# jnsquire/sregex

Measured on AMD Instinct MI355X. Metric: GB/s input scanned (whole job), gen-data stream resident in HBM, higher is better.
Workload: dtype u8; 1 GPU; configs[1]: /[a-z]+@[a-z]+\.[a-z]+/ Pike first-match + captures; 1 stream x 4.00 GiB gen-data (abccc.. + 'aaabbccb'); bytes_per_gpu=4294967293, streams_per_gpu=1, segment_bytes=16896, fixup_rounds=0, matches=0, engine=scan, lineage_passes=0, world_size=1

## Files before the change

### sregex_amd/csrc/sre_hip_scan.hip

```cpp
#include <hip/hip_runtime.h>
#include <stdlib.h>
#include "sre_hip_scan.h"
#include "sre_hip_streams.h"
#include "sre_hip_tile.h"

#define SRE_HIP_PIKE_COUNT 2
#define EV_DONE 1
#define EV_POP  2
#define RC_DECLINED (-5)
#define RC_ERROR    (-1)


__global__ void
sre_k_gen_data(uint8_t *__restrict__ dst, uint64_t n, uint64_t body, const uint8_t *__restrict__ tail)
{
    const uint64_t stride = (uint64_t) gridDim.x * blockDim.x * 16;
    for (uint64_t base = ((uint64_t) blockIdx.x * blockDim.x + threadIdx.x) * 16; base < n;
         base += stride)
    {
        uint8_t  v[16];
        unsigned ph = (unsigned) (base % 5);
#pragma unroll
        for (int k = 0; k < 16; k++) {
            uint64_t i = base + k;
// ... 439 lines not shown

template <int MODE, int BITS, bool WIDE, bool GROW>
__global__ __launch_bounds__(SRE_SCAN_BLOCK, MODE == SRE_HIP_PIKE_COUNT ? SRE_COUNT_BLOCKS : SRE_FIRST_BLOCKS) void
sre_k_scan(const sre_scan_tables_t *__restrict__ tabp, sre_scan_geom_t G,
           sre_seg_summary_t *__restrict__ sum, const sre_stream_status_t *__restrict__ st_lo,
           const uint8_t *__restrict__ entry)
{
    constexpr int      TILE = SRE_SCAN_ROUND;
    constexpr int      WARM = SRE_SCAN_LINE;
    constexpr int      STRIDE = 8 / BITS;
    constexpr uint32_t ROWRAW = TILE / STRIDE * (WIDE ? 2 : 1);
    constexpr uint32_t ROWB = 2 * ROWRAW + 16;
    constexpr int      GIDX = 16 / STRIDE;
    typedef const __attribute__((address_space(3))) uint32_t *lds_u32_t;
    extern __shared__ __attribute__((aligned(16))) uint8_t lds[];
    __shared__ uint16_t clsx[BITS == 8 ? 1 : 8 / BITS][256];
    __shared__ sre_scan_tables_t Ts;

    const uint32_t tid = threadIdx.x;
    const uint32_t nst = tabp->nstates, nrows = tabp->fast_rows, nsh = tabp->nshadow;
    uint32_t *fast = reinterpret_cast<uint32_t *>(lds);
    uint8_t  *clsl = lds + nrows * SRE_FAST_ROW_BYTES;
    uint8_t  *trl = clsl + 256;
    const uint32_t tr_bytes = (nst * (tabp->ncls + 1) * 2u + 15u) & ~15u;
    uint8_t  *sfl = trl + tr_bytes;
    uint8_t  *tile = lds + (((size_t) (sfl - lds) + nst + 15u) & ~(size_t) 15u);
    RowDesc  *rows = reinterpret_cast<RowDesc *>(tile + SRE_SCAN_BLOCK * ROWB);
    (void) nrows;
    if (tid == 0) {
        Ts = *tabp;
        Ts.cls = clsl;
        Ts.state_flags = sfl;
    }
    constexpr uint32_t LDS_SLOW = 1u << 16;
    constexpr uint32_t LDS_CNT_SHIFT = 24;
    constexpr uint32_t LDS_FRESH = 1u << 17;
    const uint32_t fast_lds = (uint32_t) (uintptr_t) (__attribute__((address_space(3))) uint8_t *) lds;
    const uint32_t trap_lds = fast_lds + nst * SRE_FAST_ROW_BYTES;
    const uint32_t shadow_lds = trap_lds + SRE_FAST_ROW_BYTES;
    auto to_lds = [fast_lds, trap_lds](uint32_t g) -> uint32_t {
        if (g & SRE_FAST_SLOW) return trap_lds | LDS_SLOW;
        return (fast_lds + (g & ~(SRE_FAST_ROW_BYTES - 1)))
               | (((g >> SRE_FAST_CNT_SHIFT) & SRE_FAST_CNT_MASK) << LDS_CNT_SHIFT)
               | ((MODE == SRE_HIP_PIKE_COUNT && (g & SRE_FAST_EVT)) ? (128u << LDS_CNT_SHIFT) : 0u)
               | ((MODE == SRE_HIP_PIKE_COUNT && (g & SRE_FAST_NEXT_FRESH)) ? LDS_FRESH : 0u);
    };
    for (uint32_t i = tid; i < nst * 64; i += SRE_SCAN_BLOCK) {
        uint4 e = reinterpret_cast<const uint4 *>(tabp->fast)[i];
        e.x = to_lds(e.x);
        e.y = to_lds(e.y);
        e.z = to_lds(e.z);
        e.w = to_lds(e.w);
        reinterpret_cast<uint4 *>(fast)[i] = e;
    }
    fast[nst * 256 + tid] = trap_lds | LDS_SLOW;
    for (uint32_t q = 0; q < nsh; q++) {
        const uint32_t s = tabp->shadow_state[q], addr = shadow_lds + q * SRE_FAST_ROW_BYTES;
        const uint32_t gl = tabp->fast[s * 256 + tid];
        fast[(nst + 1 + q) * 256 + tid] = (gl & SRE_FAST_STABLE) ? addr : to_lds(gl);
    }
    for (uint32_t i = tid; i < nst * (tabp->ncls + 1); i += SRE_SCAN_BLOCK) {
        reinterpret_cast<uint16_t *>(trl)[i] = tabp->trans2[i];
    }
    for (uint32_t i = tid; i < tabp->nstates; i += SRE_SCAN_BLOCK) sfl[i] = tabp->state_flags[i];
    clsl[tid] = tabp->cls[tid];
    if (BITS != 8) {
#pragma unroll
        for (int u = 0; u < 8 / BITS; u++) clsx[u][tid] = (uint16_t) ((uint32_t) tabp->cls[tid] << (BITS * u + (WIDE ? 2 : 0)));
    }
    __syncthreads();
    const sre_scan_tables_t &T = Ts;

    const uint64_t g = (uint64_t) blockIdx.x * SRE_SCAN_BLOCK + tid;
    bool           active = g < G.nsegs;
    uint32_t       sidx = 0;
    uint64_t       k = 0;
    int64_t        lo_s = -2;
    if (active) {
        uint32_t a = 0, b = G.nstreams;
        while (b - a > 1) {
            uint32_t m = (a + b) >> 1;
            if (geom_first(G, m) <= g) a = m; else b = m;
        }
        sidx = a;
        k = g - geom_first(G, a);
        if (st_lo != nullptr) {
            lo_s = st_lo[sidx].done ? -1 : st_lo[sidx].first_bad;
            if (lo_s < 0 || (int64_t) k < lo_s) active = false;
        }
    }

    Walk w;
    w.T = &T;
    w.tr2 = reinterpret_cast<const uint16_t *>(trl);
    w.data = nullptr;
    w.n = 0;
    w.st = 0;
    w.ev_kind = 0;
    w.ev_state = w.ev_sym = 0;
    w.ev_pos = w.ev_sp = -1;
    w.ev_apos = -1;
    w.ev_astate = 0;
    w.cur_sp = -1;
    w.warm_lo = 0;
    w.anchor_pos = -1;
    w.anchor_state = 0;
    w.lm_state = w.lm_sym = 0;
    w.lm_pos = w.lm_sp = w.lm_apos = -1;
    w.lm_astate = 0;
    w.count = 0;
    w.term_pos = -1;
    w.fl = 0;

    int64_t  seg_a = 0, seg_b = 0;
    uint32_t s_in = 0, seed = 0;
    int64_t  in_pe_pos = -1;
    uint32_t in_pe_state = 0, in_pe_sym = 0;
    bool     last_seg = false, warm = false;
    RowDesc mine;
    mine.addr = 0;
    mine.lo = 0;
    mine.hi16 = -1;
    if (active) {
        w.data = geom_ptr(G, sidx);
        w.n = (int64_t) geom_len(G, sidx);
        seg_a = (int64_t) k * G.seg_bytes;
        seg_b = seg_a + G.seg_bytes;
        const uint64_t nseg = geom_first(G, sidx + 1) - geom_first(G, sidx);
        last_seg = (k + 1 == nseg);
        if (seg_b > w.n) seg_b = w.n;
        if (last_seg && G.sentry != nullptr && (G.sentry[sidx] & SRE_SENTRY_NO_EOF)) w.fl |= F_NO_EOF;

        if (k == 0) {
            w.st = G.sentry != nullptr ? SRE_SENTRY_STATE(G.sentry[sidx])
                   : (G.flags & SRE_GEOM_CONTINUES) ? G.entry_state : T.init[G.init_variant];
            w.cur_sp = 0;
        } else if (lo_s >= 0 && (int64_t) k == lo_s) {
            const sre_seg_summary_t &c = sum[g - 1];
            w.st = c.s_out & ~SRE_STATE_SKIP;
            w.set(F_SKIP_NEXT, MODE == SRE_HIP_PIKE_COUNT && (c.s_out & SRE_STATE_SKIP) != 0);
            w.cur_sp = c.cur_sp;
            if (c.flags & SRE_SUM_PENDING) {
                w.fl |= F_HAS_EV;
                w.ev_state = c.pe_state;
                w.ev_sym = c.pe_sym;
                w.ev_pos = c.pe_pos;
                w.ev_sp = c.pe_sp;
                w.ev_apos = c.pe_apos;
                w.ev_astate = c.pe_astate;
                w.ev_kind = (uint8_t) (w.tr2[c.pe_state * (T.ncls + 1) + c.pe_sym] >> 8);
                if (MODE == SRE_HIP_PIKE_COUNT) {
                    w.fl |= F_IN_PENDING;
                    in_pe_pos = c.pe_pos;
                    in_pe_state = c.pe_state;
                    in_pe_sym = c.pe_sym;
                }
            }
        } else if (entry != nullptr && entry[g] != 0xffu) {
            w.st = entry[g];
            if (MODE == SRE_HIP_PIKE_COUNT && lo_s > 0 && (T.state_flags[w.st] & 1)) {
                const sre_seg_summary_t &c = sum[geom_first(G, sidx) + lo_s - 1];
                if (c.flags & SRE_SUM_PENDING) {
                    w.fl |= F_HAS_EV | F_IN_PENDING;
                    w.ev_state = c.pe_state;
                    w.ev_sym = c.pe_sym;
                    w.ev_pos = c.pe_pos;
                    w.ev_sp = c.pe_sp;
                    w.ev_apos = -1;
                    w.ev_astate = 0;
                    w.ev_kind = (uint8_t) (w.tr2[c.pe_state * (T.ncls + 1) + c.pe_sym] >> 8);
                    in_pe_pos = c.pe_pos;
                    in_pe_state = c.pe_state;
                    in_pe_sym = c.pe_sym;
                }
            }
        } else {
            warm = true;
            seed = T.init[0];
            if (lo_s > 0) {
                const sre_seg_summary_t &c = sum[geom_first(G, sidx) + lo_s - 1];
                const uint32_t           cs = c.s_out & ~SRE_STATE_SKIP;
                if (cs != 0) {
                    if (!(MODE == SRE_HIP_PIKE_COUNT && (T.state_flags[cs] & 1))) {
                        seed = cs;
                    } else if (c.flags & SRE_SUM_PENDING) {
                        seed = cs;
                        w.fl |= F_HAS_EV;
                        w.ev_state = c.pe_state;
                        w.ev_sym = c.pe_sym;
                        w.ev_pos = c.pe_pos;
                        w.ev_sp = c.pe_sp;
                        w.ev_apos = -1;
                        w.ev_astate = 0;
                        w.ev_kind = (uint8_t) (w.tr2[c.pe_state * (T.ncls + 1) + c.pe_sym] >> 8);
                    }
                }
            }
            w.st = seed;
        }
        w.warm_lo = seg_a >= (int64_t) WARM ? seg_a - (int64_t) WARM : 0;
        s_in = w.st | (MODE == SRE_HIP_PIKE_COUNT && w.f(F_SKIP_NEXT) ? SRE_STATE_SKIP : 0u);
        mine.addr = (uint64_t) reinterpret_cast<uintptr_t>(w.data) + (uint64_t) (seg_a - WARM);
        mine.lo = warm ? (seg_a >= WARM ? 0 : (int32_t) (WARM - seg_a)) : WARM;
        mine.hi16 = (int32_t) (WARM + (seg_b - seg_a)) - 16;
    }
    rows[tid] = mine;

    int64_t  fcA_pos = -1, fcB_pos = -1, fc_sp0 = -1;
    uint32_t fcA_len = 0, fcA_s0 = 0, fcB_len = 0, fcB_s0 = 0;
    int64_t  lz_pos = -1;
    uint32_t lz_s0 = 0;
    auto note_span = [&](int64_t pos, uint32_t len, uint32_t s0, uint32_t cnt, bool warm_round) {
        w.fl &= ~F_HAS_EV;
        if (warm_round) return;
        if (w.f(F_SP_DIRTY)) {
            fcA_pos = fcB_pos;
            fcA_len = fcB_len;
            fcA_s0 = fcB_s0;
        } else {
            fc_sp0 = w.cur_sp;
            fcA_pos = -1;
        }
        fcB_pos = pos;
        fcB_len = len;
        fcB_s0 = s0;
        if (w.f(F_PEND_LAZY)) {
            fcB_pos = lz_pos;
            fcB_len = len + (w.f(F_LZ_GROUP) ? 16u : (uint32_t) TILE);
            fcB_s0 = lz_s0;
        }
        w.fl |= F_SP_DIRTY;
        w.count += cnt;
    };
    constexpr bool any_fresh = GROW;
    auto fast_span_done = [&](int64_t pos, uint32_t len, uint32_t s0, uint32_t sum, bool fresh1, bool warm_round) {
        if (!any_fresh) {
            if (sum) note_span(pos, len, s0, sum, warm_round);
            return;
        }
        if (sum == 0) {
            w.fl &= ~F_PEND_LAZY;
            return;
        }
        if (sum & 127u) note_span(pos, len, s0, sum & 127u, warm_round);
        else if (sum) w.fl &= ~F_HAS_EV;
        if (fresh1) {
            w.fl |= F_PEND_LAZY;
            w.set(F_LZ_GROUP, len == 16u);
            lz_pos = pos;
            lz_s0 = s0;
        } else {
            w.fl &= ~F_PEND_LAZY;
        }
    };
    auto settle = [&]() {
        if (MODE != SRE_HIP_PIKE_COUNT || !(w.fl & (F_SP_DIRTY | F_PEND_LAZY))) return;
        if (w.f(F_SP_DIRTY)) {
            int64_t sp0 = fc_sp0;
            if (fcA_pos >= 0) sp0 = resolve_fast_span(&T, w.tr2, w.data, fcA_pos, fcA_len, fcA_s0, -1, -1, 0, 0).sp;
            const SpanResult r = resolve_fast_span(&T, w.tr2, w.data, fcB_pos, fcB_len, fcB_s0, sp0, w.ev_pos, w.ev_state, w.ev_sym);
            if (r.last_pos >= 0) {
                w.fl |= F_LM_VALID;
                w.lm_pos = r.last_pos;
                w.lm_state = r.last_state;
                w.lm_sym = r.last_sym;
                w.lm_sp = r.last_sp;
                const bool anchored = r.last_sp < fcB_pos && r.last_pos - fcB_pos <= 256 && fcB_pos >= seg_a;
                w.lm_apos = anchored ? fcB_pos : (int64_t) -1;
                w.lm_astate = anchored ? fcB_s0 : 0u;
            }
            w.cur_sp = r.sp;
            w.fl &= ~F_SP_DIRTY;
        }
        if (w.f(F_PEND_LAZY)) {
            const SpanResult r = resolve_fast_span(&T, w.tr2, w.data, lz_pos, w.f(F_LZ_GROUP) ? 16u : (uint32_t) TILE, lz_s0,
                                                   -1, -1, 0, 0);
            w.fl &= ~F_PEND_LAZY;
            if (r.pend_pos >= 0) {
                w.fl |= F_HAS_EV;
                w.ev_pos = r.pend_pos;
                w.ev_state = r.pend_state;
                w.ev_sym = r.pend_sym;
                w.ev_kind = (uint8_t) (w.tr2[r.pend_state * (T.ncls + 1) + r.pend_sym] >> 8);
                w.ev_sp = w.cur_sp;
                const bool anchored = w.cur_sp < lz_pos && lz_pos >= seg_a;
                w.ev_apos = anchored ? lz_pos : (int64_t) -1;
                w.ev_astate = anchored ? lz_s0 : 0u;
            }
        }
    };

    constexpr uint32_t SU_UNSET = 0xffffffffu;
    uint32_t           su = SU_UNSET, run_off = 0;
    static_assert(SRE_SCAN_MAX_SHADOWS == 2, "two shadow rows");
    const uint32_t sh_st0 = nsh > 0 ? tabp->shadow_state[0] : 0xffffu, sh_st1 = nsh > 1 ? tabp->shadow_state[1] : 0xffffu;
    const uint32_t sh_ad0 = shadow_lds, sh_ad1 = shadow_lds + SRE_FAST_ROW_BYTES;
    const uint32_t     two = 2;
    (void) two;

    const uint32_t nrounds = WARM / TILE + G.seg_bytes / TILE;
    const uint32_t lag = (tid >> 5) & 1u;
    constexpr uint32_t DIST = SRE_SCAN_PREFETCH;
    __syncthreads();
    auto round = [&](const uint32_t s, uint4 (&regs)[4]) __attribute__((always_inline)) {
        __builtin_amdgcn_fence(__ATOMIC_ACQ_REL, "wavefront");
        __builtin_amdgcn_wave_barrier();
        tile_store<BITS, WIDE>(regs, tile, clsx, tid, s);
        __builtin_amdgcn_fence(__ATOMIC_ACQ_REL, "wavefront");
        __builtin_amdgcn_wave_barrier();
        if (s + DIST <= nrounds) tile_fetch(regs, rows, tid, s + DIST);

        if (s < lag || s - lag >= nrounds) return;
        const uint32_t r = s - lag;
        const bool     warm_round = (r < WARM / TILE);
        if (!active || w.f(F_FINISHED) || (warm_round && !warm)) return;
        const int64_t base = seg_a - WARM + (int64_t) r * TILE;
        if (base >= seg_b || base < 0) return;
        w.anchor_pos = warm_round ? -1 : base;
        w.anchor_state = w.st;

        constexpr int ROWW = (ROWRAW + 3) / 4;
        uint32_t      roww[ROWW < 4 ? 4 : ROWW];
        {
            const uint8_t *src = tile + tid * ROWB + (r & 1u) * ROWRAW;
            if (ROWW >= 4) {
#pragma unroll
                for (int x = 0; x < ROWW / 4; x++) {
                    const uint4 v = *reinterpret_cast<const uint4 *>(src + 16 * x);
                    roww[4 * x] = v.x; roww[4 * x + 1] = v.y; roww[4 * x + 2] = v.z; roww[4 * x + 3] = v.w;
                }
            } else if (ROWW == 2) {
                const uint2 v = *reinterpret_cast<const uint2 *>(src);
                roww[0] = v.x; roww[1] = v.y;
            } else {
                roww[0] = *reinterpret_cast<const uint32_t *>(src);
            }
        }
        if (base + TILE <= seg_b && !(MODE == SRE_HIP_PIKE_COUNT && w.f(F_SKIP_NEXT))) {
            uint32_t t = fast_lds + w.st * SRE_FAST_ROW_BYTES, cnt = 0;
            if (MODE != SRE_HIP_PIKE_COUNT && !warm_round) {
                const uint32_t sha = w.st == sh_st0 ? sh_ad0 : w.st == sh_st1 ? sh_ad1 : 0u;
                if (!w.f(F_SHADOW)) {
                    if (sha) {
                        w.fl |= F_SHADOW;
                        run_off = (uint32_t) (base - seg_a);
                    } else if (su == SU_UNSET) {
                        su = (uint32_t) (base - seg_a);
                    }
                }
                if (w.f(F_SHADOW)) t = sha;
            }
#pragma unroll
            for (int j = 0; j < TILE * BITS / 8; j++) {
                uint32_t a;
                if (WIDE) {
                    a = (j & 1) ? add_w0_w<1>(t, roww[j >> 1]) : add_w0_w<0>(t, roww[j >> 1]);
                } else {
                    const uint32_t wj = roww[j >> 2];
                    const uint32_t ix = (j & 3) == 0 ? byte_x4<0>(wj, two) : (j & 3) == 1 ? byte_x4<1>(wj, two)
                                      : (j & 3) == 2 ? byte_x4<2>(wj, two) : byte_x4<3>(wj, two);
                    a = add_w0_w<2>(t, ix);
                }
                t = *(lds_u32_t) (uintptr_t) a;
                if (MODE == SRE_HIP_PIKE_COUNT) cnt = add_b3(cnt, t);
            }
            if (!(t & LDS_SLOW)) {
                const uint32_t ridx = ((t & 0xffffu) - fast_lds) / SRE_FAST_ROW_BYTES;
                if (MODE == SRE_HIP_PIKE_COUNT) fast_span_done(base, TILE, w.st, cnt, (t & LDS_FRESH) != 0, warm_round);
                w.st = MODE == SRE_HIP_PIKE_COUNT ? ridx : ridx <= nst ? ridx : ridx == nst + 1 ? sh_st0 : sh_st1;
                if (MODE != SRE_HIP_PIKE_COUNT && w.f(F_SHADOW) && ridx <= nst) {
                    w.fl &= ~F_SHADOW;
                    if (su == SU_UNSET) su = (uint32_t) (base - seg_a);
                }
                if (r + 1 == WARM / TILE) {
                    s_in = w.st | (MODE == SRE_HIP_PIKE_COUNT && w.f(F_SKIP_NEXT) ? SRE_STATE_SKIP : 0u);
                    settle();
                    w.cur_sp = -1;
                    if (w.f(F_HAS_EV)) w.ev_sp = -1;
                    if (w.st == 0) w.fl |= F_FINISHED;
                    if (MODE == SRE_HIP_PIKE_COUNT) {
                        w.set(F_IN_PENDING, w.f(F_HAS_EV));
                        in_pe_pos = w.ev_pos;
                        in_pe_state = w.ev_state;
                        in_pe_sym = w.ev_sym;
                    }
                }
                return;
            }
        }
        if (MODE != SRE_HIP_PIKE_COUNT && !warm_round) {
            w.fl &= ~F_SHADOW;
            if (su == SU_UNSET) su = (uint32_t) (base - seg_a);
        }
#pragma unroll 1
        for (uint32_t q = 0; q < TILE / 16; q++) {
            const int64_t gp = base + q * 16;
            if (gp >= seg_b || w.f(F_FINISHED)) break;
            const int64_t g_end = gp + 16 <= seg_b ? gp + 16 : seg_b;
            bool          exact = (g_end != gp + 16) || (MODE == SRE_HIP_PIKE_COUNT && w.f(F_SKIP_NEXT));
            uint32_t      t = fast_lds + w.st * SRE_FAST_ROW_BYTES, cnt = 0;
            if (!exact) {
                constexpr int GW = GIDX * (WIDE ? 2 : 1) / 4;
                uint32_t      gw[GW];
                const uint32_t *gsrc = reinterpret_cast<const uint32_t *>(tile + tid * ROWB + (r & 1u) * ROWRAW) + q * GW;
#pragma unroll
                for (int x = 0; x < GW; x++) gw[x] = gsrc[x];
#pragma unroll
                for (int j = 0; j < GIDX; j++) {
                    const uint32_t ix = WIDE ? (gw[j >> 1] >> ((j & 1) * 16)) & 0xffffu
                                             : ((gw[j >> 2] >> ((j & 3) * 8)) & 0xffu) << 2;
                    t = *(lds_u32_t) (uintptr_t) ((t & 0xffffu) + ix);
                    if (MODE == SRE_HIP_PIKE_COUNT) cnt += t >> LDS_CNT_SHIFT;
                }
                exact = (t & LDS_SLOW) != 0;
            }
            if (exact) {
                settle();
                slow_run<MODE>(w, gp, g_end, warm_round, seed);
            } else {
                const uint32_t st1 = ((t & 0xffffu) - fast_lds) / SRE_FAST_ROW_BYTES;
                if (MODE == SRE_HIP_PIKE_COUNT) fast_span_done(gp, 16, w.st, cnt, (t & LDS_FRESH) != 0, warm_round);
                w.st = st1;
            }
        }
        if (r + 1 == WARM / TILE) {
            s_in = w.st | (MODE == SRE_HIP_PIKE_COUNT && w.f(F_SKIP_NEXT) ? SRE_STATE_SKIP : 0u);
            settle();
            w.cur_sp = -1;
            if (w.f(F_HAS_EV)) w.ev_sp = -1;
            if (w.st == 0) w.fl |= F_FINISHED;
            if (MODE == SRE_HIP_PIKE_COUNT) {
                w.set(F_IN_PENDING, w.f(F_HAS_EV));
                in_pe_pos = w.ev_pos;
                in_pe_state = w.ev_state;
                in_pe_sym = w.ev_sym;
            }
        }
    
    };
    uint4 regs[4];
    tile_fetch(regs, rows, tid, 0);
    if (DIST == 1) {
        for (uint32_t s = 0; s <= nrounds; s++) round(s, regs);
    } else {
        uint4 regs2[4];
        if (nrounds >= 1) tile_fetch(regs2, rows, tid, 1);
        for (uint32_t s = 0; s <= nrounds; s += 2) {
            round(s, regs);
            if (s + 1 <= nrounds) round(s + 1, regs2);
        }
    }

    if (!active) return;

    if (last_seg && !w.f(F_FINISHED) && !(G.flags & SRE_GEOM_NO_EOF) && !w.f(F_NO_EOF)) {
        settle();
        w.anchor_pos = -1;
        slow_run<MODE>(w, w.n, w.n + 1, false, 0);
    }
    settle();

    sre_seg_summary_t out;
    {
        const uint32_t seg_len = (uint32_t) (seg_b - seg_a);
        if (MODE == SRE_HIP_PIKE_COUNT || (w.f(F_FINISHED) && su == SU_UNSET)) su = 0;
        out.stable_until = su == SU_UNSET ? seg_len : su;
        out.stable_from = (MODE != SRE_HIP_PIKE_COUNT && w.f(F_SHADOW)) ? run_off : seg_len;
    }
    out.s_in = w.f(F_UNRESOLVED) ? 0xffffffffu : s_in;
    out.s_out = w.st | (MODE == SRE_HIP_PIKE_COUNT && w.f(F_SKIP_NEXT) ? SRE_STATE_SKIP : 0u);
    out.flags = 0;
    out.pad = 0;
    out.count = w.count;
    out.term_pos = w.term_pos;
    out.cur_sp = w.cur_sp;
    if (w.f(F_FINISHED) && w.term_pos >= 0) out.flags |= SRE_SUM_TERM;
    if (w.f(F_ERROR)) out.flags |= SRE_SUM_ERROR;
    if (w.f(F_HAS_EV)) out.flags |= SRE_SUM_PENDING;
    if (w.f(F_LM_VALID)) out.flags |= SRE_SUM_LASTEV;
    if (MODE == SRE_HIP_PIKE_COUNT && w.f(F_IN_PENDING)) out.flags |= SRE_SUM_IN_PENDING;
    if (MODE != SRE_HIP_PIKE_COUNT && out.stable_until == G.seg_bytes && !last_seg) out.flags |= SRE_SUM_STABLE;
    out.in_pe_pos = in_pe_pos;
    out.in_pe_state = in_pe_state;
    out.in_pe_sym = in_pe_sym;
    out.pe_state = w.ev_state;
    out.pe_sym = w.ev_sym;
    out.pe_pos = w.ev_pos;
    out.pe_sp = w.ev_sp;
    out.lm_state = w.lm_state;
    out.lm_sym = w.lm_sym;
    out.lm_pos = w.lm_pos;
    out.lm_sp = w.lm_sp;
    out.lm_apos = w.lm_apos;
    out.lm_astate = w.lm_astate;
    out.pe_apos = w.ev_apos;
    out.pe_astate = w.ev_astate;
    sum[g] = out;
    if (MODE != SRE_HIP_PIKE_COUNT && G.digest != nullptr) {
        sre_seg_digest_t dg;
        dg.s_in = out.s_in;
        dg.s_out = out.s_out;
        dg.bits = ((out.flags & SRE_SUM_TERM) ? 2u : 0u) | ((out.flags & SRE_SUM_LASTEV) ? 4u : 0u) | (out.cur_sp >= 0 ? 8u : 0u)
                  | ((out.flags & SRE_SUM_STABLE) ? 0u : 16u);
        dg.count = (uint32_t) out.count;
        G.digest[g] = dg;
    }
}


#define SRE_FN_CHUNK 256u

template <int BITS>
__global__ __launch_bounds__(256) void
sre_k_seg_functions(const sre_scan_tables_t *__restrict__ tabp, sre_scan_geom_t G,
                    const sre_stream_status_t *__restrict__ status, uint8_t *__restrict__ fn)
{
    constexpr int STRIDE = 8 / BITS;
    constexpr int GIDX = 16 / STRIDE;
    typedef const __attribute__((address_space(3))) uint32_t *lds_u32_t;
    extern __shared__ __attribute__((aligned(16))) uint8_t lds[];
    __shared__ uint16_t clsx[BITS == 8 ? 1 : 8 / BITS][256];
    const uint32_t tid = threadIdx.x, nst = tabp->nstates, nsym = tabp->ncls + 1;
    uint32_t *fast = reinterpret_cast<uint32_t *>(lds);
    uint8_t  *clsl = lds + (nst + 1) * SRE_FAST_ROW_BYTES;
    uint16_t *tr2 = reinterpret_cast<uint16_t *>(clsl + 256);
    constexpr uint32_t LDS_SLOW = 1u << 16;
    const uint32_t fast_lds = (uint32_t) (uintptr_t) (__attribute__((address_space(3))) uint8_t *) lds;
    const uint32_t trap_lds = fast_lds + nst * SRE_FAST_ROW_BYTES;
    for (uint32_t i = tid; i < nst * 256; i += 256) {
        const uint32_t gl = tabp->fast[i];
        fast[i] = (gl & SRE_FAST_SLOW) ? (trap_lds | LDS_SLOW) : fast_lds + (gl & ~(SRE_FAST_ROW_BYTES - 1));
    }
    fast[nst * 256 + tid] = trap_lds | LDS_SLOW;
    clsl[tid] = tabp->cls[tid];
    for (uint32_t i = tid; i < nst * nsym; i += 256) tr2[i] = tabp->trans2[i];
    if (BITS != 8) {
#pragma unroll
        for (int u = 0; u < 8 / BITS; u++) clsx[u][tid] = (uint16_t) ((uint32_t) tabp->cls[tid] << (BITS * u + 2));
    }
    __syncthreads();

    const uint32_t lane = tid & 63u;
    const uint64_t g = (uint64_t) blockIdx.x * 4 + (tid >> 6);
    if (g >= G.nsegs) return;
    const uint32_t s = stream_of(G, g);
    const uint64_t k = g - geom_first(G, s);
    if (status[s].done || (int64_t) k < status[s].first_bad) return;
    if (lane >= nst) {
        fn[g * 64 + lane] = 0;
        return;
    }
    const uint8_t *data = geom_ptr(G, s);
    const int64_t  n = (int64_t) geom_len(G, s);
    int64_t        p = (int64_t) k * G.seg_bytes, seg_b = p + G.seg_bytes;
    if (seg_b > n) seg_b = n;
    uint32_t cur = lane;
    const bool count_mode = tabp->mode == SRE_HIP_PIKE_COUNT;
    auto exact = [&](int64_t from, int64_t to) {
        if (!count_mode) {
            for (int64_t q = from; q < to; q++) cur = tr2[cur * nsym + clsl[data[q]]] & 0xffu;
            return;
        }
        int64_t  pend = -1;
        uint32_t pkind = 0, guard = 0;
        for (int64_t q = from; q < to; q++) {
            const uint32_t sym = clsl[data[q]];
            const uint32_t t2 = tr2[cur * nsym + sym];
            if (t2 >> 8) {
                pend = q;
                pkind = t2 >> 8;
            }
            cur = t2 & 0xffu;
            if (cur != 0) continue;
            int64_t sp = q + 1;
            if (pend >= 0) {
                const bool    pop = pkind == EV_POP || pkind == SRE_DEV_EV_POP_FULL;
                const bool    empty = pkind == EV_POP || pkind == SRE_DEV_EV_DONE_EMPTY;
                const int64_t e = pop ? pend : pend + 1;
                sp = empty ? e + 1 : e;
            } else if (++guard < 2) {
                sp = q;
            }
            if (pend >= 0) guard = 0;
            if (sp < 1) sp = 1;
            if (sp > n) sp = n;
            cur = tabp->init[restart_variant_of(*tabp, data[sp - 1])];
            pend = -1;
            q = sp - 1;
        }
    };
    for (; p + 16 <= seg_b; p += 16) {
        const sre_u32x4 v = *reinterpret_cast<const __attribute__((address_space(1))) sre_u32x4_unaligned *>(
            reinterpret_cast<uintptr_t>(data + p));
        const uint32_t words[4] = {v.x, v.y, v.z, v.w};
        uint32_t       t = fast_lds + cur * SRE_FAST_ROW_BYTES;
#pragma unroll
        for (int j = 0; j < GIDX; j++) {
            uint32_t ix = 0;
#pragma unroll
            for (int u = 0; u < STRIDE; u++) {
                const int      b = j * STRIDE + u;
                const uint32_t c = (words[b >> 2] >> ((b & 3) * 8)) & 0xffu;
                ix |= BITS == 8 ? c << 2 : (uint32_t) clsx[u][c];
            }
            t = *(lds_u32_t) (uintptr_t) ((t & 0xffffu) + ix);
        }
        if (t & LDS_SLOW) exact(p, p + 16);
        else cur = ((t & 0xffffu) - fast_lds) / SRE_FAST_ROW_BYTES;
    }
    exact(p, seg_b);
    fn[g * 64 + lane] = (uint8_t) cur;
}

// ... 1769 lines not shown
```

### sregex_amd/csrc/sre_hip_tile.h

```cpp
#ifndef SRE_HIP_TILE_H
#define SRE_HIP_TILE_H

#include <hip/hip_runtime.h>
#include "sre_hip_scan.h"

namespace {

struct __attribute__((aligned(16))) RowDesc {
    uint64_t addr;
    int32_t  lo;
    int32_t  hi16;
};

typedef uint32_t sre_u32x4 __attribute__((ext_vector_type(4)));
typedef sre_u32x4 __attribute__((aligned(1))) sre_u32x4_unaligned;

__device__ inline void
tile_fetch(uint4 (&regs)[4], const RowDesc *rows, uint32_t tid, uint32_t stage)
{
    const uint32_t wbase = (tid & ~63u) + (stage & 1u) * 32u, lane = tid & 63u;
    const int32_t  line_off = (int32_t) ((stage >> 1) * SRE_SCAN_LINE);
#pragma unroll
    for (uint32_t i = 0; i < 4; i++) {
        const uint32_t piece = i * 64 + lane;
        const uint32_t row = wbase + piece / 8, col = piece % 8;
        const int32_t  off = line_off + (int32_t) (col * 16);
        const uint4    d = *reinterpret_cast<const uint4 *>(&rows[row]);
        sre_u32x4      v = {0, 0, 0, 0};
        if ((off >= (int32_t) d.z) & (off <= (int32_t) d.w)) {
            const uint64_t a = (((uint64_t) d.y << 32) | d.x) + (uint64_t) (int64_t) off;
            v = *reinterpret_cast<const __attribute__((address_space(1))) sre_u32x4_unaligned *>(a);
        }
        regs[i] = make_uint4(v.x, v.y, v.z, v.w);
    }
}

template <int BITS, bool WIDE>
__device__ inline void
tile_store(const uint4 (&regs)[4], uint8_t *tile, const uint16_t (*clsx)[256], uint32_t tid, uint32_t stage)
{
    constexpr int      STRIDE = 8 / BITS;
    constexpr uint32_t HALFB = SRE_SCAN_ROUND / STRIDE * (WIDE ? 2 : 1);
    constexpr uint32_t ROWB = 2 * HALFB + 16;
    constexpr uint32_t PIECEB = HALFB / 4;
    const uint32_t wbase = (tid & ~63u) + (stage & 1u) * 32u, lane = tid & 63u;
#pragma unroll
    for (uint32_t i = 0; i < 4; i++) {
        const uint32_t piece = i * 64 + lane;
        const uint32_t row = wbase + piece / 8, col = piece % 8;
        const uint32_t words[4] = {regs[i].x, regs[i].y, regs[i].z, regs[i].w};
        uint8_t       *dst = tile + row * ROWB + col * PIECEB;
        if (BITS == 8) {
            *reinterpret_cast<uint4 *>(dst) = regs[i];
        } else {
            constexpr int NIDX = 16 / STRIDE;
            constexpr int PERW = WIDE ? 2 : 4;
            uint32_t      out[NIDX / PERW];
#pragma unroll
            for (int k = 0; k < NIDX; k++) {
                uint32_t v = 0;
#pragma unroll
                for (int u = 0; u < STRIDE; u++) {
                    const int      b = k * STRIDE + u;
                    const uint32_t c = (words[b >> 2] >> ((b & 3) * 8)) & 0xffu;
                    v |= (uint32_t) clsx[u][c];
                }
                if (k % PERW) out[k / PERW] |= v << ((k % PERW) * (32 / PERW)); else out[k / PERW] = v;
            }
            constexpr int NW = NIDX / PERW;
            if (PIECEB == 4) *reinterpret_cast<uint32_t *>(dst) = out[0];
            else if (PIECEB == 8) *reinterpret_cast<uint2 *>(dst) = make_uint2(out[0], out[1 % NW]);
            else *reinterpret_cast<uint4 *>(dst) = make_uint4(out[0], out[1 % NW], out[2 % NW], out[3 % NW]);
        }
    }
}

constexpr uint32_t SRE_TILE2_ROWB = SRE_SCAN_ROUND + 16;

__device__ inline void
tile2_fetch(uint4 (&regs)[4], const RowDesc *rows, uint32_t tid, uint32_t stage)
{
    const uint32_t wbase = (tid & ~63u) + (stage & 1u) * 32u, lane = tid & 63u;
    const int32_t  line_off = (int32_t) ((stage >> 1) * SRE_SCAN_LINE);
#pragma unroll
    for (uint32_t i = 0; i < 4; i++) {
        const uint32_t row = wbase + (lane >> 2) + 16u * (i >> 1), col = (lane & 3u) + 4u * (i & 1u);
        const int32_t  off = line_off + (int32_t) (col * 16);
        const uint4    d = *reinterpret_cast<const uint4 *>(&rows[row]);
        sre_u32x4      v = {0, 0, 0, 0};
        if ((off >= (int32_t) d.z) & (off <= (int32_t) d.w)) {
            const uint64_t a = (((uint64_t) d.y << 32) | d.x) + (uint64_t) (int64_t) off;
            v = *reinterpret_cast<const __attribute__((address_space(1))) sre_u32x4_unaligned *>(a);
        }
        regs[i] = make_uint4(v.x, v.y, v.z, v.w);
    }
}

__device__ inline void
tile2_store(const uint4 (&regs)[4], uint4 (&hold)[2], uint8_t *tile, uint32_t tid, uint32_t stage)
{
    const uint32_t wave = tid & ~63u, lane = tid & 63u, h = stage & 1u;
    const uint32_t rnew = wave + h * 32u + (lane >> 2), rold = wave + (1u - h) * 32u + (lane >> 2);
    const uint32_t col = (lane & 3u) * 16u;
    *reinterpret_cast<uint4 *>(tile + rnew * SRE_TILE2_ROWB + col) = regs[0];
    *reinterpret_cast<uint4 *>(tile + (rnew + 16u) * SRE_TILE2_ROWB + col) = regs[2];
    *reinterpret_cast<uint4 *>(tile + rold * SRE_TILE2_ROWB + col) = hold[0];
    *reinterpret_cast<uint4 *>(tile + (rold + 16u) * SRE_TILE2_ROWB + col) = hold[1];
    hold[0] = regs[1];
    hold[1] = regs[3];
}

}

#endif
```

Before: 5458 GB/s.

## Add uniform-stride fast path for tile fetch and OR3 class packing in tile store

Adds a per-wave setup that detects when the 64 rows a wave reads are evenly strided from a common base. For the stages where every piece is in bounds, a simplified fetch replaces the per-piece row-descriptor loads and bounds checks with scalar base plus stride addressing. It also adds a specialised tile_store path for 2-bit wide tables that combines class lookups with v_or3_b32. This cuts per-round VALU and LDS-descriptor work, but adds setup cost, register pressure and a second fetch code path.

Result: slower. 5312 GB/s (-2.7%).

```diff
diff --git a/sregex_amd/csrc/sre_hip_scan.hip b/sregex_amd/csrc/sre_hip_scan.hip
--- a/sregex_amd/csrc/sre_hip_scan.hip
+++ b/sregex_amd/csrc/sre_hip_scan.hip
@@ -765,13 +765,19 @@
     const uint32_t lag = (tid >> 5) & 1u;
     constexpr uint32_t DIST = SRE_SCAN_PREFETCH;
     __syncthreads();
+    constexpr bool MID = MODE != SRE_HIP_PIKE_COUNT && BITS == 2 && WIDE;
+    TileMid        mid;
+    if (MID) tile_mid_setup(mid, rows, tid);
     auto round = [&](const uint32_t s, uint4 (&regs)[4]) __attribute__((always_inline)) {
         __builtin_amdgcn_fence(__ATOMIC_ACQ_REL, "wavefront");
         __builtin_amdgcn_wave_barrier();
-        tile_store<BITS, WIDE>(regs, tile, clsx, tid, s);
+        tile_store<BITS, WIDE, MID>(regs, tile, clsx, tid, s);
         __builtin_amdgcn_fence(__ATOMIC_ACQ_REL, "wavefront");
         __builtin_amdgcn_wave_barrier();
-        if (s + DIST <= nrounds) tile_fetch(regs, rows, tid, s + DIST);
+        if (s + DIST <= nrounds) {
+            if (MID && tile_mid_stage(mid, s + DIST)) tile_fetch_mid(regs, mid, s + DIST);
+            else tile_fetch(regs, rows, tid, s + DIST);
+        }
 
         if (s < lag || s - lag >= nrounds) return;
         const uint32_t r = s - lag;
diff --git a/sregex_amd/csrc/sre_hip_tile.h b/sregex_amd/csrc/sre_hip_tile.h
--- a/sregex_amd/csrc/sre_hip_tile.h
+++ b/sregex_amd/csrc/sre_hip_tile.h
@@ -35,7 +35,93 @@
     }
 }
 
-template <int BITS, bool WIDE>
+struct TileMid {
+    uint64_t base;
+    uint32_t d8;
+    uint32_t s_first, s_count;
+    uint32_t off;
+};
+
+__device__ inline uint64_t
+tile_uniform64(uint64_t v)
+{
+    const uint32_t lo = (uint32_t) __builtin_amdgcn_readfirstlane((int) (uint32_t) v);
+    const uint32_t hi = (uint32_t) __builtin_amdgcn_readfirstlane((int) (uint32_t) (v >> 32));
+    return ((uint64_t) hi << 32) | lo;
+}
+
+__device__ inline void
+tile_mid_setup(TileMid &m, const RowDesc *rows, uint32_t tid)
+{
+    const uint32_t wave = tid & ~63u, lane = tid & 63u;
+    const int32_t  c16 = (int32_t) ((lane & 7u) * 16u);
+    int32_t        lf = 0, ll = 0x7fffffff;
+    uint64_t       a[8];
+#pragma unroll
+    for (uint32_t q = 0; q < 8; q++) {
+        const uint4   d = *reinterpret_cast<const uint4 *>(&rows[wave + q * 8u + (lane >> 3)]);
+        const int32_t lo = (int32_t) d.z, hi = (int32_t) d.w;
+        const int32_t f = lo > c16 ? (lo - c16 + (int32_t) SRE_SCAN_LINE - 1) / (int32_t) SRE_SCAN_LINE : 0;
+        const int32_t l = hi >= c16 ? (hi - c16) / (int32_t) SRE_SCAN_LINE : -1;
+        lf = f > lf ? f : lf;
+        ll = l < ll ? l : ll;
+        a[q] = (((uint64_t) d.y << 32) | d.x) + (uint64_t) (int64_t) c16;
+    }
+    uint64_t base = a[0];
+#pragma unroll
+    for (int x = 32; x >= 1; x >>= 1) {
+        const uint64_t o = ((uint64_t) (uint32_t) __shfl_xor((int) (base >> 32), x) << 32) | (uint32_t) __shfl_xor((int) base, x);
+        const int32_t  of = __shfl_xor(lf, x), ol = __shfl_xor(ll, x);
+        base = o < base ? o : base;
+        lf = of > lf ? of : lf;
+        ll = ol < ll ? ol : ll;
+    }
+    const uint64_t d0 = a[1] - a[0];
+    const uint64_t d8 = tile_uniform64(d0);
+    bool ok = (d8 >> 28) == 0 && ((a[0] - base) >> 31) == 0;
+#pragma unroll
+    for (uint32_t q = 1; q < 8; q++) ok = ok && a[q] == a[0] + q * d8;
+    if (!__all(ok)) {
+        lf = 1;
+        ll = 0;
+    }
+    m.base = tile_uniform64(base);
+    m.d8 = (uint32_t) d8;
+    m.s_first = (uint32_t) __builtin_amdgcn_readfirstlane(2 * lf);
+    m.s_count = (uint32_t) __builtin_amdgcn_readfirstlane(ll >= lf ? 2 * (ll - lf + 1) : 0);
+    m.off = (uint32_t) (a[0] - base);
+}
+
+__device__ inline bool
+tile_mid_stage(const TileMid &m, uint32_t stage)
+{
+    return stage - m.s_first < m.s_count;
+}
+
+__device__ inline void
+tile_fetch_mid(uint4 (&regs)[4], const TileMid &m, uint32_t stage)
+{
+    typedef const __attribute__((address_space(1))) uint8_t *gptr_t;
+    const uint64_t b = m.base + (uint64_t) (stage >> 1) * SRE_SCAN_LINE + (uint64_t) ((stage & 1u) * 4u) * m.d8;
+    uint32_t       off = m.off;
+    asm volatile("" : "+v"(off));
+#pragma unroll
+    for (uint32_t i = 0; i < 4; i++) {
+        const gptr_t    p = reinterpret_cast<gptr_t>(b + (uint64_t) i * m.d8);
+        const sre_u32x4 v = *reinterpret_cast<const __attribute__((address_space(1))) sre_u32x4_unaligned *>(p + off);
+        regs[i] = make_uint4(v.x, v.y, v.z, v.w);
+    }
+}
+
+__device__ inline uint32_t
+or3_u32(uint32_t a, uint32_t b, uint32_t c)
+{
+    uint32_t r;
+    asm("v_or3_b32 %0, %1, %2, %3" : "=v"(r) : "v"(a), "v"(b), "v"(c));
+    return r;
+}
+
+template <int BITS, bool WIDE, bool OR32 = false>
 __device__ inline void
 tile_store(const uint4 (&regs)[4], uint8_t *tile, const uint16_t (*clsx)[256], uint32_t tid, uint32_t stage)
 {
@@ -52,6 +138,21 @@
         uint8_t       *dst = tile + row * ROWB + col * PIECEB;
         if (BITS == 8) {
             *reinterpret_cast<uint4 *>(dst) = regs[i];
+        } else if (OR32) {
+            static_assert(!OR32 || (BITS == 2 && WIDE), "the 32-bit ORs are written for four indices a piece, two a word");
+            uint32_t out[2];
+#pragma unroll
+            for (int m = 0; m < 2; m++) {
+                uint32_t x[2];
+#pragma unroll
+                for (int h = 0; h < 2; h++) {
+                    const uint32_t wd = words[2 * m + h];
+                    x[h] = or3_u32(clsx[0][wd & 0xffu], clsx[1][(wd >> 8) & 0xffu], clsx[2][(wd >> 16) & 0xffu])
+                           | (uint32_t) clsx[3][wd >> 24];
+                }
+                out[m] = x[0] | (x[1] << 16);
+            }
+            *reinterpret_cast<uint2 *>(dst) = make_uint2(out[0], out[1]);
         } else {
             constexpr int NIDX = 16 / STRIDE;
             constexpr int PERW = WIDE ? 2 : 4;
```
